# lxjeffffff/PagedAttention-Based-Transformer-Decoder-Inference-Framework

Hardware: AMD Instinct MI355X
Metric: decode tokens/sec at batch=64 seq_len=8192; % HBM-roofline (1/2/4/8 GPU) (higher is better)
Workload: dtype int8 GEMM (i32 acc) + fp16 KV attention (fp32 acc); 1 GPU; C3: INT8 decoder (MFMA i8 matmuls + fp16 paged attention), 24-layer/16-head/d=128, batch 64, KV context 8192, page 16; strong scaling: 64 rows over 1 GPU(s); global_batch=64, batch_per_gpu=64, seq_len=8192, page_size=16, parallelism=single GPU (no collective)

## Files before the change

pagedattention-based-transformer-decoder-inference-framework_amd/csrc/gemm_impl.hpp:

```cpp
#pragma once

#include "common.hpp"
#include "fp8.hpp"
#include "gemm.hpp"
#include "ln_wave.hpp"

namespace llm {

struct KvAppend {
  const int32_t* pos;
  const int32_t* page_table;
  const int32_t* rows;
  _Float16* k_pool;
  _Float16* v_pool;
  int num_beams, max_tiles, TS, num_pages, H, D;
  size_t page_stride;
  int fp8;
  float k_inv, v_inv;
};

struct GemmArgs {
  const uint8_t* A;
  int lda;
  int a_packed;
  const uint8_t* B;
  int M, N, K, KS;
  const float* sa;
  const float* sw;
  const float* bias;
  int act;
  float* C;
  int32_t* acc_out;
  int c_cols;
  int c_ld;
  _Float16* c16;
  KvAppend kv;
  unsigned long long* stamps;
  const float* ln_x;
  const _Float16* ln_emb;
  const int32_t* ln_tok;
  int ln_V;
  const float* ln_g;
  const float* ln_b;
  float ln_eps;
  uint8_t* act_out;
  float* sa_out;
  int partial;
  int w_keep;
  int xcd_map;
  unsigned* seam;
  int seam_n;
  int qdiag;
  int ksplit2;
};

__host__ __device__ constexpr int ln_row_stride(int K, int esize) { return K * esize + 32; }

__device__ __forceinline__ unsigned long long phase_clock() {
  unsigned long long t;
  asm volatile("s_memrealtime %0\n\ts_waitcnt lgkmcnt(0)" : "=s"(t)::"memory");
  return t;
}


template <int MT, int WAVES, int NT = 1>
constexpr int gemm_unroll() {
  return (MT >= 4 ? 2 : 4) * (WAVES == 4 ? 2 : 1) / (NT >= 4 ? 2 : 1);
}

__device__ __forceinline__ float apply_act(float y, int act) {
  if (act == LLM_ACT_RELU) return fmaxf(y, 0.f);
  if (act == LLM_ACT_GELU) return 0.5f * y * (1.f + erff(y * 0.70710678118654752f));
  return y;
}

enum class GemmKind { I8, F16 };

template <GemmKind KIND>
struct GemmTraits;
template <>
struct GemmTraits<GemmKind::I8> {
  static constexpr int KSTEP = 64, ESIZE = 1;
  using acc_t = i32x4;
  using elem_t = int32_t;
};
template <>
struct GemmTraits<GemmKind::F16> {
  static constexpr int KSTEP = 32, ESIZE = 2;
  using acc_t = f32x4;
  using elem_t = float;
};

template <GemmKind KIND, int ROWS, int WAVES>
__device__ __forceinline__ void ln_prologue(const GemmArgs& a, int m0, uint8_t* alds,
                                            float* sa_lds) {
  constexpr int ESIZE = GemmTraits<KIND>::ESIZE;
  constexpr int CPL = 8;
  const int lane = lane_id();
  const int w = wave_id_uniform();
  const int K = a.K;
  const int K4 = K >> 2;
  const int stride = ln_row_stride(K, ESIZE);
  const bool do_ln = a.ln_g != nullptr;
  LnRow<CPL> gm, bt;
  ln_wave_load(a.ln_g, K4, do_ln, gm);
  ln_wave_load(a.ln_b, K4, do_ln, bt);
  for (int r0 = w; r0 < ROWS; r0 += 2 * WAVES) {
    LnRow<CPL> x[2];
#pragma unroll
    for (int q = 0; q < 2; ++q) {
      const int r = r0 + q * WAVES;
      const int m = m0 + r;
      const bool ok = r < ROWS && m < a.M;
      if (a.ln_emb)
        ln_wave_load_f16(ok ? ln_embed_row(a.ln_emb, a.ln_tok, m, a.ln_V, K) : a.ln_emb, K4, ok,
                         x[q]);
      else
        ln_wave_load(a.ln_x + (size_t)m * K, K4, ok, x[q]);
    }
#pragma unroll
    for (int q = 0; q < 2; ++q) {
      const int r = r0 + q * WAVES;
      if (r >= ROWS) break;
      const bool mok = m0 + r < a.M;
      float am;
      if (do_ln) {
        am = ln_wave_compute(x[q], gm, bt, K, a.ln_eps);
      } else {
        am = 0.f;
#pragma unroll
        for (int j = 0; j < CPL; ++j)
#pragma unroll
          for (int e = 0; e < 4; ++e) am = fmaxf(am, fabsf(x[q].v[j][e]));
        am = ln_wave_max(am);
      }
      uint8_t* rowp = alds + (size_t)r * stride;
      if constexpr (KIND == GemmKind::I8) {
        const float scale = 127.f / (am + 1e-6f);
#pragma unroll
        for (int j = 0; j < CPL; ++j) {
          const int c = 64 * j + lane;
          if (c < K4)
            *reinterpret_cast<uint32_t*>(rowp + 4 * c) = mok ? ln_quant4(x[q].v[j], scale) : 0u;
        }
        if (lane == 0) sa_lds[r] = mok ? 1.0f / scale : 0.f;
      } else {
#pragma unroll
        for (int j = 0; j < CPL; ++j) {
          const int c = 64 * j + lane;
          if (c < K4)
            *reinterpret_cast<ln_f16x4*>(rowp + 8 * c) =
                mok ? ln_half4(x[q].v[j]) : ln_f16x4{0, 0, 0, 0};
        }
      }
    }
  }
}

__device__ __forceinline__ void seam_wait(unsigned* ctr, int n) {
  if (threadIdx.x == 0) {
    unsigned spins = 0;
    while (__hip_atomic_load(&ctr[0], __ATOMIC_RELAXED, __HIP_MEMORY_SCOPE_AGENT) < (unsigned)n) {
      __builtin_amdgcn_s_sleep(8);
      if (++spins > (1u << 21)) {
        __hip_atomic_store(&ctr[2], 1u, __ATOMIC_RELAXED, __HIP_MEMORY_SCOPE_AGENT);
        break;
      }
    }
    __builtin_amdgcn_fence(__ATOMIC_ACQUIRE, "agent");
  }
  __syncthreads();
}

template <GemmKind KIND, int MT, int NT, int WAVES, int DIAG = 0, int PRO = 0, int SEAM = 0>
__device__ __forceinline__ void gemm_tile(const GemmArgs& a, int bx, int by, int bz, int nz,
                                          int gx) {
  using Tr = GemmTraits<KIND>;
  using acc_t = typename Tr::acc_t;
  constexpr int KSTEP = Tr::KSTEP;
  constexpr int kUnroll = gemm_unroll<MT, WAVES, NT>();
  using elem_t = typename Tr::elem_t;
  using RedT = elem_t[MT * NT][4][64];
  extern __shared__ __attribute__((aligned(16))) uint8_t gemm_smem[];
  RedT* red;
  if constexpr (PRO == 0) {
    __shared__ elem_t red_static[WAVES][MT * NT][4][64];
    red = red_static;
  } else {
    red = reinterpret_cast<RedT*>(gemm_smem);
  }
  constexpr int ROWS_ = 16 * MT;
  const int a_stride = ln_row_stride(a.K, Tr::ESIZE);
  uint8_t* alds = gemm_smem;
  float* sa_lds = reinterpret_cast<float*>(gemm_smem + (size_t)ROWS_ * a_stride);

  const int lane = lane_id();
  const int w = wave_id_uniform();
  const int nt0 = bx * NT;
  const int m0 = by * 16 * MT;
  unsigned long long* stamp =
      a.stamps ? a.stamps + ((size_t)by * gx + bx) * 48 : nullptr;
  if (stamp && lane == 0) stamp[w] = phase_clock();
  const int wr = (w + bx) % WAVES;
  const int kz0 = (int)((bz * a.KS) / nz);
  const int kzn = (int)(((bz + 1) * a.KS) / nz) - kz0;
  const int ks0 = kz0 + (wr * kzn) / WAVES;
  const int ks1 = kz0 + ((wr + 1) * kzn) / WAVES;
  const int ntiles = (a.N + 15) >> 4;

  const int arow_lane = lane & 15;
  const int kgrp = lane >> 4;
  const bool apk = a.a_packed;
  const uint32_t a_bytes = apk ? (uint32_t)(((a.M + 15) / 16) * a.KS * 1024u)
                               : (uint32_t)((size_t)a.M * a.lda * Tr::ESIZE);
  const auto arsrc = __builtin_amdgcn_make_buffer_rsrc((void*)a.A, (short)0, a_bytes, 0x00020000);
  const uint32_t a_kstride = apk ? 1024u : (uint32_t)(KSTEP * Tr::ESIZE);
  const uint32_t a_kgrp_off = apk ? 0u : (uint32_t)(kgrp * (KSTEP / 4) * Tr::ESIZE);
  uint32_t a_row_off[MT];
#pragma unroll
  for (int mt = 0; mt < MT; ++mt) {
    const int row = m0 + mt * 16 + arow_lane;
    a_row_off[mt] = row >= a.M ? 0xFFFFFFF0u
                    : apk ? (uint32_t)((((m0 >> 4) + mt) * a.KS) * 1024u + lane * 16)
                          : (uint32_t)((size_t)row * a.lda * Tr::ESIZE);
  }
  const uint8_t* bbase = a.B + (size_t)nt0 * a.KS * 1024;
  const uint32_t b_bytes = (uint32_t)(min(NT, ntiles - nt0) * a.KS * 1024u);
  uint32_t b_lane_off[NT];
#pragma unroll
  for (int j = 0; j < NT; ++j) b_lane_off[j] = (uint32_t)j * a.KS * 1024u + lane * 16;
  const auto brsrc = __builtin_amdgcn_make_buffer_rsrc((void*)bbase, (short)0, b_bytes, 0x00020000);

  acc_t acc[MT][NT];
#pragma unroll
  for (int mt = 0; mt < MT; ++mt)
#pragma unroll
    for (int j = 0; j < NT; ++j) acc[mt][j] = acc_t{0, 0, 0, 0};

  struct Batch {
    u32x4 b[kUnroll][NT];
    u32x4 af[kUnroll][MT];
  };
  auto issue = [&](Batch& bt, int ks, bool do_a = true, bool do_b = true) {
#pragma unroll
    for (int u = 0; u < kUnroll; ++u) {
      const int kk = ks + u;
      const bool ok = kk < ks1;
#pragma unroll
      for (int j = 0; j < NT; ++j) {
        if (!do_b) break;
        const uint32_t boff = ok ? b_lane_off[j] + (uint32_t)kk * 1024u : 0xFFFFFFF0u;
        bt.b[u][j] = a.w_keep ? __builtin_amdgcn_raw_buffer_load_b128(brsrc, boff, 0, 0)
                              : __builtin_amdgcn_raw_buffer_load_b128(brsrc, boff, 0, 2);
      }
#pragma unroll
      for (int mt = 0; mt < MT; ++mt) {
        if (!do_a) break;
        if constexpr (PRO != 0) {
          const int r = mt * 16 + arow_lane;
          bt.af[u][mt] = ok ? *reinterpret_cast<const u32x4*>(alds + (size_t)r * a_stride +
                                                             16 * (4 * kk + kgrp))
                            : u32x4{0u, 0u, 0u, 0u};
          continue;
        }
        const uint32_t koff = (uint32_t)kk * a_kstride + a_kgrp_off;
        const uint32_t aoff = (ok && a_row_off[mt] != 0xFFFFFFF0u) ? a_row_off[mt] + koff : 0xFFFFFFF0u;
        if constexpr ((DIAG & 1) != 0)
          bt.af[u][mt] = u32x4{aoff, 0u, 0u, 0u};
        else
          bt.af[u][mt] = __builtin_amdgcn_raw_buffer_load_b128(arsrc, aoff, 0, 0);
      }
    }
  };
  auto compute = [&](const Batch& bt) {
#pragma unroll
    for (int u = 0; u < kUnroll; ++u) {
#pragma unroll
      for (int mt = 0; mt < MT; ++mt) {
        if constexpr (KIND == GemmKind::I8) {
#pragma unroll
          for (int j = 0; j < NT; ++j)
            acc[mt][j] = __builtin_amdgcn_mfma_i32_16x16x64_i8(
                __builtin_bit_cast(i32x4, bt.af[u][mt]), __builtin_bit_cast(i32x4, bt.b[u][j]),
                acc[mt][j], 0, 0, 0);
        } else if constexpr (KIND == GemmKind::F16) {
#pragma unroll
          for (int j = 0; j < NT; ++j)
            acc[mt][j] = __builtin_amdgcn_mfma_f32_16x16x32_f16(
                __builtin_bit_cast(f16x8, bt.af[u][mt]), __builtin_bit_cast(f16x8, bt.b[u][j]),
                acc[mt][j], 0, 0, 0);
        }
      }
    }
  };

  constexpr int ROWS = 16 * MT, COLS = 16 * NT, NTHR = WAVES * 64;
  constexpr int EPT = (ROWS * COLS + NTHR - 1) / NTHR;
  const KvAppend& kv = a.kv;
  const int hid = kv.H * kv.D;
  float e_scale[EPT], e_bias[EPT];
  int e_pos[EPT], e_br[EPT], e_page[EPT];
#pragma unroll
  for (int e = 0; e < EPT; ++e) {
    const int o = threadIdx.x + e * NTHR;
    const int m = m0 + o / COLS;
    const int n = nt0 * 16 + o % COLS;
    const bool valid = o < ROWS * COLS && m < a.M && n < a.N;
    e_scale[e] = 1.f;
    if constexpr (KIND == GemmKind::I8) {
      if (!PRO && valid && a.sa) e_scale[e] *= a.sa[m];
      if (valid && a.sw) e_scale[e] *= a.sw[n];
    }
    e_bias[e] = valid && a.bias && (!a.ksplit2 || bz == 0) ? a.bias[n] : 0.f;
    const bool kvcol = valid && kv.k_pool && n >= hid;
    e_pos[e] = kvcol ? kv.pos[m] : -1;
    e_br[e] = kvcol ? (kv.rows ? kv.rows[m] : m) : -1;
  }

  Batch b0, b1;
  bool b1_pre = false;
  if constexpr (PRO != 0) {
    bool pre = true;
#if LLM_TUNING
    pre = (a.qdiag & 2) == 0;
#endif
    if (pre && ks0 < ks1) issue(b0, ks0, false, true);
    if (pre && ks0 + kUnroll < ks1) {
      issue(b1, ks0 + kUnroll, false, true);
      b1_pre = true;
    }
    if constexpr (SEAM != 0) seam_wait(a.seam, a.seam_n);
#if LLM_TUNING
    if ((a.qdiag & 1) == 0)
#endif
    ln_prologue<KIND, ROWS_, WAVES>(a, m0, alds, sa_lds);
    __syncthreads();
    if constexpr (KIND == GemmKind::I8) {
#pragma unroll
      for (int e = 0; e < EPT; ++e) {
        const int o = threadIdx.x + e * NTHR;
        if (o < ROWS * COLS) e_scale[e] *= sa_lds[o / COLS];
      }
    }
    if (a.act_out && bx == 0) {
      const int KS = a.KS;
      for (int i = threadIdx.x; i < ROWS_ * KS * 4; i += NTHR) {
        const int r = i / (KS * 4), g = i % (KS * 4);
        const int m = m0 + r;
        if (m >= a.M) continue;
        const size_t off = ((size_t)((m >> 4) * KS + (g >> 2)) * 64 + (m & 15) + 16 * (g & 3)) * 16;
        *reinterpret_cast<u32x4*>(a.act_out + off) =
            *reinterpret_cast<const u32x4*>(alds + (size_t)r * a_stride + 16 * g);
      }
      if (KIND == GemmKind::I8 && a.sa_out && threadIdx.x < ROWS_ && m0 + (int)threadIdx.x < a.M)
        a.sa_out[m0 + threadIdx.x] = sa_lds[threadIdx.x];
    }
  }

  {
    int ks = ks0;
    bool b0_b = PRO == 0;
#if LLM_TUNING
    if constexpr (PRO != 0) b0_b = (a.qdiag & 2) != 0;
#endif
    if (ks < ks1) issue(b0, ks, true, b0_b);
#pragma unroll
    for (int e = 0; e < EPT; ++e) {
      const int o = threadIdx.x + e * NTHR;
      const int n = nt0 * 16 + o % COLS;
      const int p = e_pos[e], br = e_br[e];
      int page = -1;
      if (p >= 0 && br >= 0 && br < kv.num_beams && p / kv.TS < kv.max_tiles) {
        const int which = n >= 2 * hid;
        const int h = (n - hid * (1 + which)) / kv.D;
        page = kv.page_table[((size_t)br * kv.H + h) * kv.max_tiles + p / kv.TS];
        if (page >= kv.num_pages) page = -1;
      }
      e_page[e] = page;
    }
    while (ks < ks1) {
      if (ks + kUnroll < ks1) {
        issue(b1, ks + kUnroll, true, !b1_pre);
        b1_pre = false;
      }
      compute(b0);
      ks += kUnroll;
      if (ks >= ks1) break;
      if (ks + kUnroll < ks1) issue(b0, ks + kUnroll);
      compute(b1);
      ks += kUnroll;
    }
  }

  if (stamp && lane == 0) stamp[16 + w] = phase_clock();
  if constexpr ((DIAG & 2) != 0) {
    int32_t x = 0;
#pragma unroll
    for (int mt = 0; mt < MT; ++mt)
#pragma unroll
      for (int j = 0; j < NT; ++j) x ^= (int32_t)acc[mt][j][0] ^ (int32_t)acc[mt][j][3];
    if (lane == 0 && a.C) a.C[bx] = (float)x;
    if (stamp && lane == 0) stamp[32 + w] = phase_clock();
    return;
  }
  if constexpr (PRO != 0) __syncthreads();
#pragma unroll
  for (int mt = 0; mt < MT; ++mt)
#pragma unroll
    for (int j = 0; j < NT; ++j)
#pragma unroll
      for (int r = 0; r < 4; ++r) red[wr][mt * NT + j][r][lane] = acc[mt][j][r];
  __syncthreads();

#pragma unroll
  for (int e = 0; e < EPT; ++e) {
#pragma clang fp contract(off)
    const int o = threadIdx.x + e * NTHR;
    if (o >= ROWS * COLS) break;
    const int cl = o % COLS;
    const int row = o / COLS;
    const int j = cl >> 4;
    const int col = cl & 15;
    const int mt = row >> 4;
    const int rl = row & 15;
    const int src_lane = (rl >> 2) * 16 + col;
    const int reg = rl & 3;
    const int m = m0 + row;
    const int n = (nt0 + j) * 16 + col;
    if (m >= a.M || n >= a.N) continue;
    float y;
    if constexpr (KIND == GemmKind::I8) {
      int32_t s = 0;
#pragma unroll
      for (int ww = 0; ww < WAVES; ++ww) s += red[ww][mt * NT + j][reg][src_lane];
#if LLM_TUNING
      if (a.partial) {
        a.acc_out[((size_t)bz * a.M + m) * a.N + n] = s;
        continue;
      }
#endif
      if (a.acc_out) a.acc_out[(size_t)m * a.N + n] = s;
      y = (float)s * e_scale[e];
      if (a.bias) y = y + e_bias[e];
      if (a.ksplit2) {
        atomicAdd(a.C + (size_t)m * a.c_ld + n, y);
        continue;
      }
    } else {
      float s = 0.f;
#pragma unroll
      for (int ww = 0; ww < WAVES; ++ww) s += red[ww][mt * NT + j][reg][src_lane];
      y = a.bias ? s + e_bias[e] : s;
    }
    y = apply_act(y, a.act);
    if (a.C && n < a.c_cols) a.C[(size_t)m * a.c_ld + n] = y;
    if (a.c16) a.c16[a_frag_off_f16(m, n, a.N >> 5)] = (_Float16)y;
    if (e_page[e] >= 0) {
      const int which = n >= 2 * hid;
      const int i = n - hid * (1 + which);
      const int d = i % kv.D;
      const int p = e_pos[e];
      const size_t off = (size_t)e_page[e] * kv.page_stride + (size_t)(p % kv.TS) * kv.D + d;
      if (kv.fp8)
        reinterpret_cast<uint8_t*>(which ? kv.v_pool : kv.k_pool)[off] =
            (uint8_t)fp8_e4m3_byte(y, which ? kv.v_inv : kv.k_inv);
      else
        (which ? kv.v_pool : kv.k_pool)[off] = (_Float16)y;
    }
  }
  if (stamp && lane == 0) stamp[32 + w] = phase_clock();
}

template <GemmKind KIND, int MT, int NT, int WAVES, int DIAG = 0, int PRO = 0>
__global__ __launch_bounds__(WAVES * 64) void gemm_kernel(GemmArgs a) {
  int bx = blockIdx.x, by = blockIdx.y, bz = blockIdx.z;
#if LLM_TUNING
  if (a.xcd_map) {
    const int per = 8 / (int)gridDim.z;
    const int lin = blockIdx.x + gridDim.x * (blockIdx.y + gridDim.y * blockIdx.z);
    const int xcd = lin & 7;
    const int tile = (lin >> 3) * per + xcd % per;
    bz = xcd / per;
    bx = tile % (int)gridDim.x;
    by = tile / (int)gridDim.x;
  }
#endif
  gemm_tile<KIND, MT, NT, WAVES, DIAG, PRO>(a, bx, by, bz, (int)gridDim.z, (int)gridDim.x);
}

template <typename T, int EPL>
__global__ void pack_kernel(const T* __restrict__ W, T* __restrict__ P, int K, int N, int KS,
                            int ntiles) {
  const size_t idx = (size_t)blockIdx.x * blockDim.x + threadIdx.x;
  const size_t total = (size_t)ntiles * KS * 64;
  if (idx >= total) return;
  const int lane = idx & 63;
  const size_t blk = idx >> 6;
  const int ks = blk % KS;
  const int nt = blk / KS;
  const int n = nt * 16 + (lane & 15);
  const int kb = ks * (4 * EPL) + (lane >> 4) * EPL;
  T* dst = P + idx * EPL;
#pragma unroll
  for (int j = 0; j < EPL; ++j) {
    const int k = kb + j;
    dst[j] = (k < K && n < N) ? W[(size_t)k * N + n] : T(0);
  }
}

namespace {

inline int pick_nt(int N, int M) {
  if (M <= 16) return 1;
  const int ntiles = (N + 15) / 16;
  const int mblocks = (M + 63) / 64;
  return (ntiles % 2 == 0 && (ntiles / 2) * mblocks >= 192) ? 2 : 1;
}

template <GemmKind KIND, int MT, int NT, int WAVES>
size_t ln_lds_bytes(int K) {
  const size_t img = (size_t)16 * MT * ln_row_stride(K, GemmTraits<KIND>::ESIZE) + 16 * MT * 4;
  const size_t red = (size_t)WAVES * MT * NT * 4 * 64 * 4;
  return img > red ? img : red;
}
constexpr size_t kLnLdsMax = 160 * 1024;

struct GemmForm {
  int mt;
  int nt;
  int waves;
  int kslices;
  int prologue;
};

template <GemmKind KIND, int MT, int NT>
hipError_t launch_gemm_nt(const GemmArgs& a, const GemmForm& f, int mblocks, hipStream_t st) {
  const int ntiles = (a.N + 15) / 16;
  const dim3 grid((ntiles + NT - 1) / NT, mblocks, f.kslices);
  if constexpr (NT <= 2) {
    if (f.prologue) {
      const size_t lds = ln_lds_bytes<KIND, MT, NT, 8>(a.K);
      hipLaunchKernelGGL((gemm_kernel<KIND, MT, NT, 8, 0, 1>), grid, dim3(512), lds, st, a);
      return hipGetLastError();
    }
  }
  if constexpr (MT * NT * 8 <= 64) {
    if (f.waves == 8) {
      hipLaunchKernelGGL((gemm_kernel<KIND, MT, NT, 8>), grid, dim3(512), 0, st, a);
      return hipGetLastError();
    }
  }
  hipLaunchKernelGGL((gemm_kernel<KIND, MT, NT, 4>), grid, dim3(256), 0, st, a);
  return hipGetLastError();
}

template <GemmKind KIND, int MT>
hipError_t launch_gemm_mt(const GemmArgs& a, const GemmForm& f, int mblocks, hipStream_t st) {
#if LLM_TUNING
  if (f.nt == 4) return launch_gemm_nt<KIND, MT, 4>(a, f, mblocks, st);
  if (f.nt == 3) return launch_gemm_nt<KIND, MT, 3>(a, f, mblocks, st);
#endif
  return f.nt == 2 ? launch_gemm_nt<KIND, MT, 2>(a, f, mblocks, st)
                   : launch_gemm_nt<KIND, MT, 1>(a, f, mblocks, st);
}

}

namespace {

inline int pick_waves(const GemmArgs&, int) { return 8; }

struct TileChoice {
  int nt, waves, mrows;
};
inline bool narrow_tile_for(int M, int N, int K, TileChoice& t) {
  if (M <= 16 || M > 64) return false;
  const int ntiles = (N + 15) / 16;
  if (M > 32) {
    if (ntiles >= 256) return false;
    t = TileChoice{2, 8, 16};
    return true;
  }
  if (ntiles < 384) {
    t = K >= 4096 ? TileChoice{1, 8, 16} : TileChoice{1, 4, 16};
    return true;
  }
  if (ntiles < 512) {
    t = TileChoice{1, 4, 16};
    return true;
  }
  return false;
}
inline bool narrow_decode_tile(const GemmArgs& a, int kstep, TileChoice& t) {
  if ((a.ln_x && a.ln_g) || a.partial) return false;
  if (a.ksplit2 && a.M > 32 && a.M <= 64) {
    t = TileChoice{2, 8, 64};
    return true;
  }
  return narrow_tile_for(a.M, a.N, a.KS * kstep, t);
}

inline GemmForm gemm_form(const GemmArgs& a, int kstep, int nt_override = 0,
                          int waves_override = 0, int mrows_override = 0, int ks_override = 0) {
  TileChoice tc{0, 0, 0};
  const bool narrow = nt_override == 0 && waves_override == 0 && mrows_override == 0 &&
                      narrow_decode_tile(a, kstep, tc);
  if (narrow) {
    nt_override = tc.nt;
    waves_override = tc.waves;
    mrows_override = tc.mrows;
  }
  const int NT = nt_override > 0 ? nt_override : pick_nt(a.N, a.M);
  const int waves = waves_override > 0 ? waves_override : pick_waves(a, NT);
  int mrows = a.M <= 16 ? 16 : a.M <= 32 ? 32 : 64;
  if (mrows == 64 && NT == 1 && (a.N + 15) / 16 < 256 && !a.ln_x && !a.partial) mrows = 32;
  if (mrows_override > 0) mrows = mrows_override;
  GemmForm f{};
  f.mt = mrows == 16 ? 1 : mrows == 32 ? 2 : 4;
  f.nt = NT == 2 ? 2 : 1;
#if LLM_TUNING
  if ((NT == 3 || NT == 4) && !a.ln_x) f.nt = NT;
#endif
  f.prologue = a.ln_x != nullptr;
  f.waves = f.prologue || (f.mt * f.nt * 8 <= 64 && waves != 4) ? 8 : 4;
  f.kslices = a.partial ? std::max(1, ks_override) : a.ksplit2 ? 2 : 1;
  return f;
}

template <GemmKind KIND>
hipError_t launch_gemm(const GemmArgs& a_in, hipStream_t st, int nt_override = 0,
                       int waves_override = 0, int mrows_override = 0, int ks_override = 0) {
  GemmArgs a = a_in;
  const GemmForm f = gemm_form(a, GemmTraits<KIND>::KSTEP, nt_override, waves_override,
                               mrows_override, ks_override);
  const int mblocks = (a.M + 16 * f.mt - 1) / (16 * f.mt);
  const int tiles = ((a.N + 15) / 16 + f.nt - 1) / f.nt * mblocks;
  if (a.xcd_map && (f.kslices < 2 || 8 % f.kslices != 0 || (tiles * f.kslices) % 8 != 0))
    a.xcd_map = 0;
  if (f.mt == 1) return launch_gemm_mt<KIND, 1>(a, f, mblocks, st);
  if (f.mt == 2) return launch_gemm_mt<KIND, 2>(a, f, mblocks, st);
  return launch_gemm_mt<KIND, 4>(a, f, mblocks, st);
}

}
}
```

Baseline: 3794 tokens/s.

## Swap MFMA operands and vectorize GEMM epilogue into 4-wide column stores

Swaps the A and B operands of the MFMA so each lane's four accumulator registers hold four consecutive output columns instead of four rows. The cross-wave reduction buffer is restructured to store whole accumulator vectors, using a swizzled slot index to avoid LDS bank conflicts. The epilogue then handles quads of columns, using vector loads of scale and bias and vector stores to C, acc_out, c16 and the KV cache pool. Scalar fallback paths cover misaligned or ragged cases, at the cost of extra code and branching in the epilogue.

```diff
diff --git a/pagedattention-based-transformer-decoder-inference-framework_amd/csrc/gemm_impl.hpp b/pagedattention-based-transformer-decoder-inference-framework_amd/csrc/gemm_impl.hpp
--- a/pagedattention-based-transformer-decoder-inference-framework_amd/csrc/gemm_impl.hpp
+++ b/pagedattention-based-transformer-decoder-inference-framework_amd/csrc/gemm_impl.hpp
@@ -179,12 +179,12 @@
   using acc_t = typename Tr::acc_t;
   constexpr int KSTEP = Tr::KSTEP;
   constexpr int kUnroll = gemm_unroll<MT, WAVES, NT>();
-  using elem_t = typename Tr::elem_t;
-  using RedT = elem_t[MT * NT][4][64];
+  using RedT = acc_t[MT * NT][64];
+  auto red_slot = [](int l) { return (l & 48) | ((l + (l >> 4) * 4) & 15); };
   extern __shared__ __attribute__((aligned(16))) uint8_t gemm_smem[];
   RedT* red;
   if constexpr (PRO == 0) {
-    __shared__ elem_t red_static[WAVES][MT * NT][4][64];
+    __shared__ acc_t red_static[WAVES][MT * NT][64];
     red = red_static;
   } else {
     red = reinterpret_cast<RedT*>(gemm_smem);
@@ -281,13 +281,13 @@
 #pragma unroll
           for (int j = 0; j < NT; ++j)
             acc[mt][j] = __builtin_amdgcn_mfma_i32_16x16x64_i8(
-                __builtin_bit_cast(i32x4, bt.af[u][mt]), __builtin_bit_cast(i32x4, bt.b[u][j]),
+                __builtin_bit_cast(i32x4, bt.b[u][j]), __builtin_bit_cast(i32x4, bt.af[u][mt]),
                 acc[mt][j], 0, 0, 0);
         } else if constexpr (KIND == GemmKind::F16) {
 #pragma unroll
           for (int j = 0; j < NT; ++j)
             acc[mt][j] = __builtin_amdgcn_mfma_f32_16x16x32_f16(
-                __builtin_bit_cast(f16x8, bt.af[u][mt]), __builtin_bit_cast(f16x8, bt.b[u][j]),
+                __builtin_bit_cast(f16x8, bt.b[u][j]), __builtin_bit_cast(f16x8, bt.af[u][mt]),
                 acc[mt][j], 0, 0, 0);
         }
       }
@@ -295,28 +295,35 @@
   };
 
   constexpr int ROWS = 16 * MT, COLS = 16 * NT, NTHR = WAVES * 64;
-  constexpr int EPT = (ROWS * COLS + NTHR - 1) / NTHR;
+  constexpr int W = ROWS * COLS <= NTHR ? 1 : 4;
+  constexpr int QCOLS = COLS / W, QUADS = ROWS * QCOLS;
+  constexpr int QPT = (QUADS + NTHR - 1) / NTHR;
+  typedef float yv_t __attribute__((ext_vector_type(W)));
+  typedef typename Tr::elem_t sv_t __attribute__((ext_vector_type(W)));
+  typedef _Float16 hv_t __attribute__((ext_vector_type(W)));
   const KvAppend& kv = a.kv;
   const int hid = kv.H * kv.D;
-  float e_scale[EPT], e_bias[EPT];
-  int e_pos[EPT], e_br[EPT], e_page[EPT];
-#pragma unroll
-  for (int e = 0; e < EPT; ++e) {
-    const int o = threadIdx.x + e * NTHR;
-    const int m = m0 + o / COLS;
-    const int n = nt0 * 16 + o % COLS;
-    const bool valid = o < ROWS * COLS && m < a.M && n < a.N;
-    e_scale[e] = 1.f;
-    if constexpr (KIND == GemmKind::I8) {
-      if (!PRO && valid && a.sa) e_scale[e] *= a.sa[m];
-      if (valid && a.sw) e_scale[e] *= a.sw[n];
-    }
-    e_bias[e] = valid && a.bias && (!a.ksplit2 || bz == 0) ? a.bias[n] : 0.f;
-    const bool kvcol = valid && kv.k_pool && n >= hid;
-    e_pos[e] = kvcol ? kv.pos[m] : -1;
-    e_br[e] = kvcol ? (kv.rows ? kv.rows[m] : m) : -1;
-  }
-
+  auto al16 = [](const void* p) { return (reinterpret_cast<uintptr_t>(p) & (4 * W - 1)) == 0; };
+  const bool n_vec = (a.N & (W - 1)) == 0;
+  const bool sw_vec = al16(a.sw), bias_vec = al16(a.bias);
+  const uintptr_t kv_al = kv.fp8 ? W - 1 : 2 * W - 1;
+  const bool kv_vec = n_vec && (kv.D & (W - 1)) == 0 && (kv.page_stride & (W - 1)) == 0 &&
+                      (reinterpret_cast<uintptr_t>(kv.k_pool) & kv_al) == 0 &&
+                      (reinterpret_cast<uintptr_t>(kv.v_pool) & kv_al) == 0;
+  const bool all_vec = (!a.C || (al16(a.C) && (a.c_ld & (W - 1)) == 0)) &&
+                       (!a.acc_out || (al16(a.acc_out) && n_vec)) &&
+                       (!a.c16 || ((reinterpret_cast<uintptr_t>(a.c16) & (2 * W - 1)) == 0 &&
+                                   (a.N & 31) == 0)) &&
+                       (!kv.k_pool || kv_vec);
+  auto kv_page = [&](int p, int br, int n) {
+    if (p < 0 || br < 0 || br >= kv.num_beams || p / kv.TS >= kv.max_tiles) return -1;
+    const int which = n >= 2 * hid;
+    const int h = (n - hid * (1 + which)) / kv.D;
+    const int page = kv.page_table[((size_t)br * kv.H + h) * kv.max_tiles + p / kv.TS];
+    return page >= kv.num_pages ? -1 : page;
+  };
+  yv_t q_scale[QPT], q_bias[QPT];
+  int q_pos[QPT], q_br[QPT], q_page[QPT];
   Batch b0, b1;
   bool b1_pre = false;
   if constexpr (PRO != 0) {
@@ -335,13 +342,6 @@
 #endif
     ln_prologue<KIND, ROWS_, WAVES>(a, m0, alds, sa_lds);
     __syncthreads();
-    if constexpr (KIND == GemmKind::I8) {
-#pragma unroll
-      for (int e = 0; e < EPT; ++e) {
-        const int o = threadIdx.x + e * NTHR;
-        if (o < ROWS * COLS) e_scale[e] *= sa_lds[o / COLS];
-      }
-    }
     if (a.act_out && bx == 0) {
       const int KS = a.KS;
       for (int i = threadIdx.x; i < ROWS_ * KS * 4; i += NTHR) {
@@ -365,18 +365,44 @@
 #endif
     if (ks < ks1) issue(b0, ks, true, b0_b);
 #pragma unroll
-    for (int e = 0; e < EPT; ++e) {
+    for (int e = 0; e < QPT; ++e) {
       const int o = threadIdx.x + e * NTHR;
-      const int n = nt0 * 16 + o % COLS;
-      const int p = e_pos[e], br = e_br[e];
-      int page = -1;
-      if (p >= 0 && br >= 0 && br < kv.num_beams && p / kv.TS < kv.max_tiles) {
-        const int which = n >= 2 * hid;
-        const int h = (n - hid * (1 + which)) / kv.D;
-        page = kv.page_table[((size_t)br * kv.H + h) * kv.max_tiles + p / kv.TS];
-        if (page >= kv.num_pages) page = -1;
-      }
-      e_page[e] = page;
+      const int m = m0 + o / QCOLS;
+      const int n = nt0 * 16 + W * (o % QCOLS);
+      const bool valid = o < QUADS && m < a.M && n < a.N;
+      const bool whole = valid && n + W <= a.N;
+      q_scale[e] = yv_t(1.f);
+      q_bias[e] = yv_t(0.f);
+      if constexpr (KIND == GemmKind::I8) {
+        if (!PRO && valid && a.sa) q_scale[e] *= a.sa[m];
+        if (valid && a.sw) {
+          if (__builtin_expect(whole && sw_vec, 1)) {
+            q_scale[e] *= *reinterpret_cast<const yv_t*>(a.sw + n);
+          } else {
+#pragma nounroll
+            for (int i = 0; i < min(W, a.N - n); ++i) q_scale[e][i] *= a.sw[n + i];
+          }
+        }
+      }
+      if (valid && a.bias && (!a.ksplit2 || bz == 0)) {
+        if (__builtin_expect(whole && bias_vec, 1)) {
+          q_bias[e] = *reinterpret_cast<const yv_t*>(a.bias + n);
+        } else {
+#pragma nounroll
+          for (int i = 0; i < min(W, a.N - n); ++i) q_bias[e][i] = a.bias[n + i];
+        }
+      }
+      if constexpr (KIND == GemmKind::I8 && PRO != 0) {
+        if (o < QUADS) q_scale[e] *= sa_lds[o / QCOLS];
+      }
+      const bool kvq = kv.k_pool && all_vec && whole && n >= hid;
+      q_pos[e] = kvq ? kv.pos[m] : -1;
+      q_br[e] = kvq ? (kv.rows ? kv.rows[m] : m) : -1;
+    }
+#pragma unroll
+    for (int e = 0; e < QPT; ++e) {
+      const int o = threadIdx.x + e * NTHR;
+      q_page[e] = kv_page(q_pos[e], q_br[e], nt0 * 16 + W * (o % QCOLS));
     }
     while (ks < ks1) {
       if (ks + kUnroll < ks1) {
@@ -407,65 +433,114 @@
 #pragma unroll
   for (int mt = 0; mt < MT; ++mt)
 #pragma unroll
-    for (int j = 0; j < NT; ++j)
-#pragma unroll
-      for (int r = 0; r < 4; ++r) red[wr][mt * NT + j][r][lane] = acc[mt][j][r];
+    for (int j = 0; j < NT; ++j) red[wr][mt * NT + j][red_slot(lane)] = acc[mt][j];
   __syncthreads();
 
-#pragma unroll
-  for (int e = 0; e < EPT; ++e) {
+  auto kv_store = [&](int page, int p, int n, auto v) {
+    const int which = n >= 2 * hid;
+    const int d = (n - hid * (1 + which)) % kv.D;
+    const size_t off = (size_t)page * kv.page_stride + (size_t)(p % kv.TS) * kv.D + d;
+    _Float16* pool = which ? kv.v_pool : kv.k_pool;
+    const float inv = which ? kv.v_inv : kv.k_inv;
+    if constexpr (sizeof(v) == sizeof(float)) {
+      const float v0 = *reinterpret_cast<const float*>(&v);
+      if (kv.fp8)
+        reinterpret_cast<uint8_t*>(pool)[off] = (uint8_t)fp8_e4m3_byte(v0, inv);
+      else
+        pool[off] = (_Float16)v0;
+    } else if (kv.fp8) {
+      uint32_t b4 = 0;
+#pragma unroll
+      for (int i = 0; i < 4; ++i) b4 |= (fp8_e4m3_byte(v[i], inv) & 0xFFu) << (8 * i);
+      *reinterpret_cast<uint32_t*>(reinterpret_cast<uint8_t*>(pool) + off) = b4;
+    } else {
+      *reinterpret_cast<ln_f16x4*>(pool + off) = ln_half4(v);
+    }
+  };
+#pragma unroll
+  for (int e = 0; e < QPT; ++e) {
 #pragma clang fp contract(off)
     const int o = threadIdx.x + e * NTHR;
-    if (o >= ROWS * COLS) break;
-    const int cl = o % COLS;
-    const int row = o / COLS;
-    const int j = cl >> 4;
-    const int col = cl & 15;
-    const int mt = row >> 4;
-    const int rl = row & 15;
-    const int src_lane = (rl >> 2) * 16 + col;
-    const int reg = rl & 3;
+    if (o >= QUADS) break;
+    const int cl = W * (o % QCOLS);
+    const int row = o / QCOLS;
+    const int tile = (row >> 4) * NT + (cl >> 4);
+    const int slot = red_slot(((cl >> 2) & 3) * 16 + (row & 15));
     const int m = m0 + row;
-    const int n = (nt0 + j) * 16 + col;
+    const int n = nt0 * 16 + cl;
     if (m >= a.M || n >= a.N) continue;
-    float y;
+    const int cnt = min(W, a.N - n);
+    sv_t s = sv_t(0);
+#pragma unroll
+    for (int ww = 0; ww < WAVES; ++ww) {
+      if constexpr (W == 4)
+        s += red[ww][tile][slot];
+      else
+        s += sv_t(red[ww][tile][slot][cl & 3]);
+    }
+    const bool vec = all_vec && cnt == W && (n >= a.c_cols || n + W <= a.c_cols);
+    yv_t y;
     if constexpr (KIND == GemmKind::I8) {
-      int32_t s = 0;
-#pragma unroll
-      for (int ww = 0; ww < WAVES; ++ww) s += red[ww][mt * NT + j][reg][src_lane];
 #if LLM_TUNING
       if (a.partial) {
-        a.acc_out[((size_t)bz * a.M + m) * a.N + n] = s;
+        int32_t* pp = a.acc_out + ((size_t)bz * a.M + m) * a.N + n;
+        if (__builtin_expect(vec, 1)) {
+          *reinterpret_cast<sv_t*>(pp) = s;
+        } else {
+#pragma nounroll
+          for (int i = 0; i < cnt; ++i) pp[i] = s[i];
+        }
         continue;
       }
 #endif
-      if (a.acc_out) a.acc_out[(size_t)m * a.N + n] = s;
-      y = (float)s * e_scale[e];
-      if (a.bias) y = y + e_bias[e];
+      if (a.acc_out) {
+        int32_t* pa = a.acc_out + (size_t)m * a.N + n;
+        if (__builtin_expect(vec, 1)) {
+          *reinterpret_cast<sv_t*>(pa) = s;
+        } else {
+#pragma nounroll
+          for (int i = 0; i < cnt; ++i) pa[i] = s[i];
+        }
+      }
+#pragma unroll
+      for (int i = 0; i < W; ++i) {
+        y[i] = (float)s[i] * q_scale[e][i];
+        if (a.bias) y[i] = y[i] + q_bias[e][i];
+      }
       if (a.ksplit2) {
-        atomicAdd(a.C + (size_t)m * a.c_ld + n, y);
+#pragma nounroll
+        for (int i = 0; i < cnt; ++i) atomicAdd(a.C + (size_t)m * a.c_ld + n + i, y[i]);
         continue;
       }
     } else {
-      float s = 0.f;
-#pragma unroll
-      for (int ww = 0; ww < WAVES; ++ww) s += red[ww][mt * NT + j][reg][src_lane];
-      y = a.bias ? s + e_bias[e] : s;
-    }
-    y = apply_act(y, a.act);
-    if (a.C && n < a.c_cols) a.C[(size_t)m * a.c_ld + n] = y;
-    if (a.c16) a.c16[a_frag_off_f16(m, n, a.N >> 5)] = (_Float16)y;
-    if (e_page[e] >= 0) {
-      const int which = n >= 2 * hid;
-      const int i = n - hid * (1 + which);
-      const int d = i % kv.D;
-      const int p = e_pos[e];
-      const size_t off = (size_t)e_page[e] * kv.page_stride + (size_t)(p % kv.TS) * kv.D + d;
-      if (kv.fp8)
-        reinterpret_cast<uint8_t*>(which ? kv.v_pool : kv.k_pool)[off] =
-            (uint8_t)fp8_e4m3_byte(y, which ? kv.v_inv : kv.k_inv);
-      else
-        (which ? kv.v_pool : kv.k_pool)[off] = (_Float16)y;
+#pragma unroll
+      for (int i = 0; i < W; ++i) y[i] = a.bias ? s[i] + q_bias[e][i] : s[i];
+    }
+    if (a.act == LLM_ACT_RELU) {
+#pragma unroll
+      for (int i = 0; i < W; ++i) y[i] = apply_act(y[i], LLM_ACT_RELU);
+    } else if (a.act == LLM_ACT_GELU) {
+#pragma nounroll
+      for (int i = 0; i < W; ++i) y[i] = apply_act(y[i], LLM_ACT_GELU);
+    }
+    if (__builtin_expect(vec, 1)) {
+      if (a.C && n < a.c_cols) *reinterpret_cast<yv_t*>(a.C + (size_t)m * a.c_ld + n) = y;
+      if (a.c16)
+        *reinterpret_cast<hv_t*>(a.c16 + a_frag_off_f16(m, n, a.N >> 5)) = __builtin_convertvector(y, hv_t);
+      if (q_page[e] >= 0) kv_store(q_page[e], q_pos[e], n, y);
+    } else {
+      const bool kvrow = kv.k_pool != nullptr;
+      const int p = kvrow ? kv.pos[m] : -1;
+      const int br = kvrow ? (kv.rows ? kv.rows[m] : m) : -1;
+#pragma nounroll
+      for (int i = 0; i < cnt; ++i) {
+        const int ni = n + i;
+        const float yi = y[i];
+        if (a.C && ni < a.c_cols) a.C[(size_t)m * a.c_ld + ni] = yi;
+        if (a.c16) a.c16[a_frag_off_f16(m, ni, a.N >> 5)] = (_Float16)yi;
+        const int page = ni >= hid ? kv_page(p, br, ni) : -1;
+        if (page >= 0) kv_store(page, p, ni, yi);
+      }
     }
   }
   if (stamp && lane == 0) stamp[32 + w] = phase_clock();
```

After: 3812 tokens/s, median of 6. About the same (+0.5%).
